# samuel-vitorino/lm.rs

Hardware: AMD Instinct MI355X
Metric: decode tok/s + %HBM-roofline, Llama-3.2-1B Q8_0 @1/2/4/8 MI355X vs CPU ref (higher is better)
Workload: dtype int8xint8->int32, f32 combine; 1 GPU; llama-3.2-1b Q8_0 (gs=128) greedy decode, 5-token synthetic prompt then 3164 tokens, batch 1; parallelism=single GPU, image_bytes=1274634496

## Files before the change

lm.rs_amd/csrc/lmrs_api.hip:

```cpp
#include <hip/hip_runtime.h>
#include <hip/hip_ext.h>
#include <rccl/rccl.h>
#include <math.h>
#include <stdio.h>
#include <stdlib.h>
#include <string.h>

#include <algorithm>
#include <chrono>
#include <string>
#include <vector>

#include "../../include/lmrs_hip.h"
#include "lmrs_device_math.h"
#include "lmrs_format.h"
#include "lmrs_kernels.h"
#include "lmrs_score.h"
#include "lmrs_switches.h"

using namespace lmrs;

static thread_local std::string g_err;
static int fail(const std::string& m) { g_err = m; return -1; }
#define HIP_OK(expr)                                                                                     \
// ... 3 lines not shown
    } while (0)

extern "C" const char* lmrs_last_error(void) { return g_err.c_str(); }
namespace lmrs { int text_fail(const char* msg) { return fail(msg); } }

namespace {

struct DevLayer {
    const void *wqkv, *wo, *w13, *w2;
    const float *sqkv, *so, *s13, *s2;
    const float *sqkvT = nullptr, *soT = nullptr, *s13T = nullptr, *s2T = nullptr;
    const float *rms_att, *rms_post_att, *rms_pre_ffn, *rms_post_ffn;
};

}
static int prefill_alloc(lmrs_ctx* c);

struct lmrs_ctx {
    lmrs_args args{};
    Layout lay;
    int device = 0;
    hipStream_t stream = nullptr;
    char* arena = nullptr; size_t arena_bytes = 0, arena_used = 0;
    std::vector<DevLayer> layers;
    const void *emb_q = nullptr, *cls_q = nullptr; const float *emb_s = nullptr, *cls_s = nullptr, *rms_final = nullptr;
    float *x = nullptr, *q = nullptr, *k_raw = nullptr, *att_out = nullptr, *h = nullptr, *logits = nullptr, *tmp = nullptr;
    float *part_val = nullptr; int* part_idx = nullptr;
    float *k_cache = nullptr, *v_cache = nullptr, *rope = nullptr;
    float* stage = nullptr; size_t stage_floats = 0;
    uint32_t* tokens = nullptr; DevState* st = nullptr;
    unsigned long long* dbg = nullptr; int dbg_node = 0;
    unsigned long long* samp_keys = nullptr; float* samp_pairs = nullptr; void* h_pairs = nullptr; int samp_cap = 0;
    float* h_logits = nullptr; uint32_t* h_tok = nullptr; DevState* h_st = nullptr; unsigned h_st_next = 0;
    hipGraphExec_t g_steps[7][2] = {}, g_layers = nullptr;
    float* att_S = nullptr; int att_split_pos = 0;
    float *pf_x = nullptr, *pf_q = nullptr, *pf_k = nullptr, *pf_ao = nullptr, *pf_h = nullptr, *pf_xs = nullptr, *pf_t = nullptr; int8_t* pf_xq = nullptr; float* pf_att = nullptr; size_t pf_att_cap = 0;
    bool pf_ready = false;
    char *pfx_att = nullptr, *pfx_h = nullptr, *pfx_x = nullptr; size_t pfb_att = 0, pfb_h = 0, pfb_x = 0; bool pfx_owned = false;
    bool tp_prefill = false;
    float* x2 = nullptr; bool gemma_fused = false;
    hipEvent_t ev0 = nullptr, ev1 = nullptr;
    Switches sw;
    std::vector<float*> scales_t;
    int att_dim = 0, kv_dim = 0, cls_grid = 0;
    int part_stride = 0;
    bool q4 = false, f32 = false;
    int rank = 0, world = 1;
    int att_full = 0;
    int dim_l = 0, hid_l = 0, voc_l = 0;
    int d0 = 0, h0 = 0, v0 = 0, a0 = 0;
    bool rep_out = true;
    bool cls_only = false;
    ncclComm_t comm = nullptr;
    bool eager = false;
    float* part = nullptr;
    bool qpay = false; char *gq_att = nullptr, *gq_h = nullptr; size_t blk_att = 0, blk_h = 0;
    bool p2p = false, p2p_ready = false; char* xarena = nullptr; size_t xarena_bytes = 0; char* peer_base[kMaxWorld] = {};
    unsigned *xflags = nullptr, *xseq = nullptr; int* xerr = nullptr; int ex_slot = 0; bool xarena_is_ipc[kMaxWorld] = {};
    double last_fill_ms = -1.0;
    bool err_queued = false;
    int* err = nullptr; int* h_err = nullptr;
    bool qkv_att = false; unsigned long long* gran = nullptr; unsigned* seq = nullptr; int qa_max_T = 0, qa_wave_T = 0;
    int multi_k = 1;
    bool cls_tail = false; unsigned long long* part_pk = nullptr; unsigned* cls_seq = nullptr;
    int inj_fail_connect = 0, inj_stall_seg = -1; long long inj_stall_ticks = 0;
    float* sc_logits = nullptr; int sc_rows = 0; ScorePart* sc_part = nullptr; double* sc_lp = nullptr; uint32_t* sc_idx = nullptr; char* h_sc = nullptr;
    unsigned long long* tk_cand = nullptr; uint32_t* tk_cnt = nullptr; uint32_t* tk_idx = nullptr; float* tk_val = nullptr; uint32_t* tk_rank = nullptr;
    char* h_tk = nullptr; int tk_rows = 0, tk_k = 0;

    template <class T> T* alloc(size_t count) {
        size_t bytes = (count * sizeof(T) + 255) & ~(size_t)255;
        if (arena_used + bytes > arena_bytes) return nullptr;
        T* p = reinterpret_cast<T*>(arena + arena_used); arena_used += bytes; return p;
    }
};

namespace {

__global__ void advance_pos_kernel(DevState* st, unsigned* seq) { st->pos += 1; st->step_count += 1; *seq += 1u; }
__global__ void stall_kernel(long long ticks) { const long long t0 = wall_clock64(); while (wall_clock64() - t0 < ticks) __builtin_amdgcn_s_sleep(32); }

size_t pad256(size_t b) { return (b + 255) & ~(size_t)255; }

constexpr int kPrefillTokens = 512;
bool prefill_tp_shapes_ok(const lmrs_ctx* c) {
    const lmrs_args& a = c->args;
    if (c->world < 1 || c->cls_only || c->f32 || c->sw.no_batched_prefill) return false;
    if (!c->rep_out && c->dim_l % 16) return false;
    if (a.q_type != LMRS_Q8_0 && a.q_type != LMRS_Q4_0) return false;
    if (c->att_dim % 128 || c->hid_l % 128) return false;
    if (!rows_prologue_supported((int)a.dim)) return false;
    if (a.model_type == LMRS_GEMMA) { if (a.head_size != 256 || a.dim != 2304) return false; }
    else if (a.head_size != 64 && a.head_size != 96 && a.head_size != 128) return false;
    return (c->att_dim + 2 * c->kv_dim) % 16 == 0 && c->kv_dim % 4 == 0 && a.dim % 16 == 0 && c->att_full % 128 == 0 && a.hidden_dim % 128 == 0;
}
size_t prefill_tp_block(size_t n_l) { return pad256((size_t)kPrefillTokens * n_l + (size_t)kPrefillTokens * (n_l / 128) * 4); }

struct StepForm { int qa_mode = 0, split_chunks = 0; };
struct PassForm { bool skinny = false; const RowTable* rows = nullptr; int max_T = 0; float *k_cache = nullptr, *v_cache = nullptr; RowView runs{}; float* qkv = nullptr; };
StepForm step_form_for(const lmrs_ctx* c, uint32_t pos, bool merged = true) {
    StepForm f;
    if (c->att_split_pos > 0 && (int)pos >= c->att_split_pos) {
        int b = 0;
        while (b < 3 && pos >= (1024u << b)) ++b;
        f.split_chunks = 4 << b;
    } else if (merged && c->qkv_att) f.qa_mode = (int)pos < c->qa_wave_T ? 2 : ((int)pos < c->qa_max_T ? 1 : 0);
    return f;
}
int split_scratch(lmrs_ctx* c, StepForm f) {
    if (!f.split_chunks || c->att_S) return 0;
    HIP_OK(hipMalloc(reinterpret_cast<void**>(&c->att_S), attention_split_scratch_floats(c->att_dim / (int)c->args.head_size, (int)c->args.seq_len) * 4));
    return 0;
}

void rope_terms(const lmrs_args& a, uint32_t p, uint32_t j, float* fcr, float* fci) {
    static const double short_factor[48] = {
        1.08, 1.1, 1.1300000000000001, 1.2800000000000002, 1.3100000000000003, 1.4500000000000004, 1.4500000000000004,
        1.9500000000000008, 2.030000000000001, 2.4299999999999926, 2.5699999999999896, 2.9499999999999815, 3.729999999999965,
        3.869999999999962, 4.189999999999955, 4.43999999999995, 4.6399999999999455, 4.979999999999938, 5.159999999999934,
        5.279999999999932, 5.759999999999922, 5.889999999999919, 5.889999999999919, 5.969999999999917, 6.089999999999915,
        6.2799999999999105, 6.7699999999999, 6.8899999999998975, 7.109999999999893, 7.129999999999892, 7.179999999999891,
        7.289999999999889, 7.339999999999888, 7.559999999999883, 7.619999999999882, 7.69999999999988, 7.879999999999876,
        7.879999999999876, 7.879999999999876, 7.939999999999875, 7.949999999999875, 7.979999999999874, 8.19999999999987,
        8.439999999999864, 8.469999999999864, 8.589999999999861, 8.809999999999857, 8.999999999999853};
    const uint32_t head_dim = j * 2;
    float freq = 1.0f / powf(a.rope_theta, (float)head_dim / (float)a.head_size);
    float scaling_factor = 1.0f;
    if (a.model_type == LMRS_LLAMA) {
        const float wavelen = (2.0f * 3.14159265358979323846f) / freq;
        const float factor = 32.0f, low_freq_factor = 1.0f, high_freq_factor = 4.0f, old_context_len = 8192.0f;
        const float low_freq_wavelen = old_context_len / low_freq_factor;
        const float high_freq_wavelen = old_context_len / high_freq_factor;
        if (wavelen > low_freq_wavelen) freq = freq / factor;
        else if (wavelen <= low_freq_wavelen && wavelen >= high_freq_wavelen) {
            const float smooth_factor = (old_context_len / wavelen - low_freq_factor) / (high_freq_factor - low_freq_factor);
            freq = (1.0f - smooth_factor) * freq / factor + smooth_factor * freq;
        }
    }
// ... 36 lines not shown
    HIP_OK(launch_gemv_f32(g, PRO_QUANT, gemma ? EPI_STORE : EPI_RESID, c->stream));
    set_launch_tag(7);
    if (gemma) HIP_OK(launch_addnorm(c->x, c->tmp, L.rms_post_att, a.dim, a.rms_norm_eps, c->stream));
    set_launch_tag(3);
    g.wq = L.w13; g.n = a.dim; g.o = 2 * a.hidden_dim; g.xin = c->x; g.rms_w = gemma ? L.rms_pre_ffn : L.rms_post_att; g.out = c->h;
    HIP_OK(launch_gemv_f32(g, PRO_RMS_QUANT, gemma ? EPI_GELU : EPI_SWIGLU, c->stream));
    set_launch_tag(4);
    g.wq = L.w2; g.n = a.hidden_dim; g.o = a.dim; g.xin = c->h; g.out = gemma ? c->tmp : c->x;
    HIP_OK(launch_gemv_f32(g, PRO_QUANT, gemma ? EPI_STORE : EPI_RESID, c->stream));
    set_launch_tag(7);
    if (gemma) HIP_OK(launch_addnorm(c->x, c->tmp, L.rms_post_ffn, a.dim, a.rms_norm_eps, c->stream));
    return 0;
}

int enqueue_layer(lmrs_ctx* c, StepForm f, int l) {
    if (c->f32) return enqueue_layer_f32(c, f, l);
    const lmrs_args& a = c->args;
    const DevLayer& L = c->layers[l];
    const bool gemma = a.model_type == LMRS_GEMMA;
    GemvArgs g{};
    g.q4 = c->q4; g.eps = a.rms_norm_eps; g.add_unit = gemma; g.st = c->st;
    g.att_dim = c->att_dim; g.kv_dim = c->kv_dim; g.seq_len = a.seq_len; g.layer = l;
    g.wq = L.wqkv; g.ws = L.sqkv; g.n = a.dim; g.o = c->att_dim + 2 * c->kv_dim;
    g.xin = c->x; g.rms_w = L.rms_att; g.out = c->q; g.k_raw = c->k_raw; g.v_cache = c->v_cache;
    g.att_dim = c->att_dim; g.kv_dim = c->kv_dim; g.seq_len = a.seq_len; g.layer = l;
    g.dbg = c->dbg ? c->dbg + 8 * (c->dbg_node++) : nullptr;
    set_launch_tag(0);
    const bool pending = c->gemma_fused && l > 0;
    if (pending) { g.xin = c->x2; g.delta = c->tmp; g.add_w = c->layers[l - 1].rms_post_ffn; g.xout = c->x; }
    AttnArgs t{};
    t.q = c->q; t.k_raw = c->k_raw; t.k_cache = c->k_cache; t.v_cache = c->v_cache; t.rope = c->rope; t.out = c->att_out;
    t.n_heads = a.n_heads; t.n_kv_heads = a.n_kv_heads; t.head_size = a.head_size; t.seq_len = a.seq_len; t.layer = l;
    t.gemma = gemma; t.st = c->st;
    if (f.qa_mode && !f.split_chunks) {
        g.gran = c->gran + (size_t)l * (c->att_dim + 2 * c->kv_dim); g.seq = c->seq;
        t.dbg = c->dbg ? c->dbg + 8 * (c->dbg_node++) : nullptr;
        HIP_OK(launch_qkv_attn(g, pending ? PRO_ADD_RMS_QUANT : PRO_RMS_QUANT, t, c->err, c->qa_max_T, f.qa_mode == 2, c->stream));
        g.gran = nullptr; g.seq = nullptr;
    } else {
    HIP_OK(launch_gemv(g, pending ? PRO_ADD_RMS_QUANT : PRO_RMS_QUANT, EPI_QKV, c->stream));
    t.dbg = c->dbg ? c->dbg + 8 * (c->dbg_node++) : nullptr;
    set_launch_tag(1);
    if (f.split_chunks) HIP_OK(launch_attention_split(t, c->att_S, f.split_chunks, c->stream));
    else HIP_OK(launch_attention(t, c->stream));
    }
    g.delta = nullptr; g.add_w = nullptr; g.xout = nullptr;
    g.wq = L.wo; g.ws = L.so; g.n = c->att_dim; g.o = a.dim; g.xin = c->att_out; g.out = gemma ? c->tmp : c->x;
    g.dbg = c->dbg ? c->dbg + 8 * (c->dbg_node++) : nullptr;
    set_launch_tag(2);
    HIP_OK(launch_gemv(g, PRO_QUANT, gemma ? EPI_STORE : EPI_RESID, c->stream));
    set_launch_tag(7);
    if (gemma && !c->gemma_fused) HIP_OK(launch_addnorm(c->x, c->tmp, L.rms_post_att, a.dim, a.rms_norm_eps, c->stream));
    g.wq = L.w13; g.ws = L.s13; g.n = a.dim; g.o = 2 * a.hidden_dim; g.xin = c->x; g.rms_w = gemma ? L.rms_pre_ffn : L.rms_post_att; g.out = c->h;
    g.dbg = c->dbg ? c->dbg + 8 * (c->dbg_node++) : nullptr;
    if (c->gemma_fused) { g.delta = c->tmp; g.add_w = L.rms_post_att; g.xout = c->x2; }
    set_launch_tag(3);
    HIP_OK(launch_gemv(g, c->gemma_fused ? PRO_ADD_RMS_QUANT : PRO_RMS_QUANT, gemma ? EPI_GELU : EPI_SWIGLU, c->stream));
    g.delta = nullptr; g.add_w = nullptr; g.xout = nullptr;
    g.wq = L.w2; g.ws = L.s2; g.n = a.hidden_dim; g.o = a.dim; g.xin = c->h; g.out = gemma ? c->tmp : c->x;
    g.dbg = c->dbg ? c->dbg + 8 * (c->dbg_node++) : nullptr;
    set_launch_tag(4);
    HIP_OK(launch_gemv(g, PRO_QUANT, gemma ? EPI_STORE : EPI_RESID, c->stream));
    set_launch_tag(7);
    if (gemma && !c->gemma_fused) HIP_OK(launch_addnorm(c->x, c->tmp, L.rms_post_ffn, a.dim, a.rms_norm_eps, c->stream));
    return 0;
}

// ... 223 lines not shown
        ++c->ex_slot;
        x.par_bytes = (int)e.par;
        if (e.qsrc) { x.qsrc = e.qsrc; x.qn = (int)e.qn; }
        set_launch_tag(8);
        HIP_OK(e.wide ? launch_exchange_copy_push(x, c->stream) : launch_exchange_push(x, c->stream));
        return 0;
    }
    if (!c->comm) return fail("this context is a member of a lock-step shard group: drive it with lmrs_group_forward");
    NCCL_OK(ncclAllGather(e.buf + (size_t)c->rank * e.stride, e.buf, e.stride, ncclUint8, c->comm, c->stream));
    return 0;
}

int capture(lmrs_ctx* c, StepForm f, bool full, hipGraphExec_t* out, int n_steps = 1) {
    hipGraph_t graph = nullptr;
    c->dbg_node = 0;
    HIP_OK(hipStreamBeginCapture(c->stream, hipStreamCaptureModeThreadLocal));
    int rc = 0;
    if (full) { for (int k = 0; k < n_steps && !rc; ++k) rc = c->world > 1 || c->comm ? enqueue_step_sharded(c, f) : enqueue_step(c, f); }
    else {
        for (uint32_t l = 0; l < c->args.n_layers && !rc; ++l) rc = enqueue_layer(c, f, (int)l);
        if (!rc) rc = enqueue_finish_residual(c);
        if (!rc) hipLaunchKernelGGL(advance_pos_kernel, dim3(1), dim3(1), 0, c->stream, c->st, c->seq);
    }
    hipError_t e = hipStreamEndCapture(c->stream, &graph);
    if (rc) { if (graph) (void)hipGraphDestroy(graph); return -1; }
    if (e != hipSuccess) return fail(std::string("hipStreamEndCapture: ") + hipGetErrorString(e));
    e = hipGraphInstantiate(out, graph, nullptr, nullptr, 0);
    (void)hipGraphDestroy(graph);
    if (e != hipSuccess) return fail(std::string("hipGraphInstantiate: ") + hipGetErrorString(e));
    return 0;
}

hipGraphExec_t step_graph(lmrs_ctx* c, StepForm f, int k = 1) {
    hipGraphExec_t& g = c->g_steps[f.split_chunks ? __builtin_ctz(f.split_chunks) + 1 : f.qa_mode][k > 1];
    if (!g && capture(c, f, true, &g, k)) g = nullptr;
    return g;
}
int replay_steps(lmrs_ctx* c, StepForm f, int k = 1) {
    hipGraphExec_t g = step_graph(c, f, k);
    if (!g) return -1;
    HIP_OK(hipGraphLaunch(g, c->stream));
    return 0;
}
hipGraphExec_t primary_graph(const lmrs_ctx* c) { return c->g_steps[step_form_for(c, 0).qa_mode][0]; }
void capture_sharded_step(lmrs_ctx* c) {
    if (!step_graph(c, step_form_for(c, 0))) { c->eager = true; (void)hipGetLastError(); g_err.clear(); }
}
void destroy_step_graphs(lmrs_ctx* c) {
    for (auto& forms : c->g_steps) for (hipGraphExec_t& g : forms) if (g) { (void)hipGraphExecDestroy(g); g = nullptr; }
}

int upload(lmrs_ctx* c, void* dst, const uint8_t* src, size_t bytes) {
    HIP_OK(hipMemcpyAsync(dst, src, bytes, hipMemcpyHostToDevice, c->stream));
    return 0;
}
int upload_interleaved(lmrs_ctx* c, void* dst, const uint8_t* src, size_t row_bytes, size_t rows, int phase) {
    HIP_OK(hipMemcpy2DAsync(static_cast<char*>(dst) + phase * row_bytes, 2 * row_bytes, src, row_bytes, row_bytes, rows,
                            hipMemcpyHostToDevice, c->stream));
    return 0;
}

constexpr unsigned kStateSlots = 16;
int set_state(lmrs_ctx* c, uint32_t pos, uint32_t prompt_end, int win_base = -1) {
    DevState* hs = c->h_st + (c->h_st_next++ % kStateSlots);
    hs->pos = (int)pos; hs->prompt_end = (int)prompt_end; hs->step_count = 0; hs->win_base = win_base;
    HIP_OK(hipMemcpyAsync(c->st, hs, sizeof(DevState), hipMemcpyHostToDevice, c->stream));
    if (c->qkv_att || c->cls_tail) HIP_OK(hipMemsetAsync(c->err, 0, 4, c->stream));
// ... 369 lines not shown
        std::vector<float> tab((size_t)a.seq_len * a.head_size);
        for (uint32_t p = 0; p < a.seq_len; ++p)
            for (uint32_t j = 0; j < half; ++j) rope_terms(a, p, j, &tab[((size_t)p * half + j) * 2], &tab[((size_t)p * half + j) * 2 + 1]);
        HCK(hipMemcpyAsync(c->rope, tab.data(), tab.size() * 4, hipMemcpyHostToDevice, c->stream));
        HCK(hipStreamSynchronize(c->stream));
    }
    HCK(hipHostMalloc(reinterpret_cast<void**>(&c->h_logits), V * 4, hipHostMallocDefault));
    HCK(hipHostMalloc(reinterpret_cast<void**>(&c->h_tok), ((size_t)a.seq_len + 8) * 4, hipHostMallocDefault));
    HCK(hipHostMalloc(reinterpret_cast<void**>(&c->h_st), kStateSlots * sizeof(DevState), hipHostMallocDefault));
    HCK(hipHostMalloc(reinterpret_cast<void**>(&c->h_err), 4, hipHostMallocDefault));
    CK(set_state(c, 0, 0));
    HCK(hipStreamSynchronize(c->stream));
    if (a.model_type == LMRS_GEMMA && !sharded && !f32w) {
        GemvArgs q{}; q.q4 = c->q4; q.n = a.dim; q.o = c->att_dim + 2 * c->kv_dim;
        GemvArgs f = q; f.o = 2 * a.hidden_dim;
        GemvArgs k = q; k.o = cls_rows(c); k.softcap_rows = (int)a.dim;
        c->gemma_fused = gemv_is_static(q, PRO_ADD_RMS_QUANT, EPI_QKV) && gemv_is_static(f, PRO_ADD_RMS_QUANT, EPI_GELU) &&
                         gemv_is_static(k, PRO_ADD_RMS_QUANT, EPI_CLS);
    }
    {
        GemvArgs g = cls_args(c);
        c->cls_grid = f32w ? gemv_f32_grid(g, EPI_CLS) : gemv_grid(g, c->gemma_fused ? PRO_ADD_RMS_QUANT : PRO_RMS_QUANT, EPI_CLS);
        c->part_stride = (2 * c->cls_grid + 3) & ~3;
    }
    if ((!sharded || (cls_only && !group_mode)) && !f32w && sw.qkv_att != 0) {
        GemvArgs q{}; q.q4 = c->q4; q.n = a.dim; q.o = c->att_dim + 2 * c->kv_dim;
        AttnArgs t{}; t.n_heads = a.n_heads; t.n_kv_heads = a.n_kv_heads; t.head_size = a.head_size; t.gemma = a.model_type == LMRS_GEMMA;
        c->qkv_att = qkv_attn_supported(q, PRO_RMS_QUANT, t) && (!c->gemma_fused || qkv_attn_supported(q, PRO_ADD_RMS_QUANT, t)) &&
                     !(a.model_type == LMRS_GEMMA && !c->gemma_fused);
        c->qa_max_T = a.seq_len < 1024 ? (int)a.seq_len : 1024;
        if (c->qkv_att && sw.qkv_att != 1) c->qa_wave_T = qkv_attn_wave_T((int)a.head_size);
        if (c->qa_wave_T > (int)a.seq_len) c->qa_wave_T = a.head_size == 64 && a.seq_len >= 128 ? (int)a.seq_len : 0;
    }
    if (!sharded) c->multi_k = sw.steps_per_graph;
    c->cls_tail = !sharded && !f32w && V < (1u << 20) - 1 && sw.cls_tail;
    if (!sharded) {
        CK(!step_graph(c, step_form_for(c, 0)));
        CK(capture(c, StepForm{}, false, &c->g_layers));
        if (!c->dbg || sw.att_split_pos_set) c->att_split_pos = sw.att_split_pos;
        if (!c->dbg && c->qkv_att) {
            for (int mode = 1; mode <= 2; ++mode) {
                if (mode == 2 && c->qa_wave_T <= 0) continue;
                if (mode == 1 && c->qa_wave_T >= c->qa_max_T) continue;
                CK(!step_graph(c, StepForm{mode, 0}));
                if (c->multi_k > 1) CK(!step_graph(c, StepForm{mode, 0}, c->multi_k));
            }
        }
    } else if (c->comm) {
        capture_sharded_step(c);
    }
    if (sharded) c->att_split_pos = sw.att_split_pos;
    if (c->tp_prefill && c->comm && (c->world > 1 || c->comm) && !c->cls_only) CK(prefill_alloc(c));
#undef CK
#undef HCK
    *out = c;
    if (bytes_consumed) *bytes_consumed = lay.end;
    return 0;
}

static void topk_free(lmrs_ctx* c) {
    for (void** p : {(void**)&c->tk_cand, (void**)&c->tk_cnt, (void**)&c->tk_idx, (void**)&c->tk_val, (void**)&c->tk_rank}) if (*p) { (void)hipFree(*p); *p = nullptr; }
    if (c->h_tk) { (void)hipHostFree(c->h_tk); c->h_tk = nullptr; }
    c->tk_rows = c->tk_k = 0;
}

extern "C" void lmrs_destroy(lmrs_ctx* c) {
// ... 1527 lines not shown
    return 0;
}

extern "C" int lmrs_debug_inject(lmrs_ctx* c, int what, int a, int b) {
    if (!c) return fail("ctx is NULL");
    if (what == 0) { c->inj_fail_connect = 1; return 0; }
    if (what == 1) {
        if (!(c->comm || c->p2p)) return fail("not a row-sharded context");
        HIP_OK(hipSetDevice(c->device));
        HIP_OK(hipStreamSynchronize(c->stream));
        destroy_step_graphs(c);
        c->eager = true; c->inj_stall_seg = a; c->inj_stall_ticks = (long long)b * 100;
        return 0;
    }
    return fail("unknown injection");
}

extern "C" int lmrs_debug_gemm_tile(uint32_t n, uint32_t o, uint32_t n_tok, int q4, int* tile_rows, int* tile_tokens, int* waves) {
    if (!tile_rows || !tile_tokens || !waves) return fail("NULL argument");
    if (n == 0 || n % 256 || o == 0 || o % 16 || n_tok == 0) return fail("lmrs_debug_gemm_tile: n must be a positive multiple of 256, o of 16");
    *tile_rows = *tile_tokens = *waves = 0;
    if (n_tok >= 48) { const GemmTile t = gemm_q8_ring_tile((int)n, (int)o, (int)n_tok, q4 != 0); *tile_rows = t.tm; *tile_tokens = t.tn; *waves = t.waves; }
    return 0;
}

extern "C" int lmrs_step_info(const lmrs_ctx* c, uint32_t pos, int* n_launches, double* algo_bytes) {
    if (!c) return fail("ctx is NULL");
    const lmrs_args& a = c->args;
    const double bpe = c->f32 ? 4.0 - 4.0 / 128.0 : (c->q4 ? 0.5 : 1.0), dim = a.dim, att = c->att_dim, kv = c->kv_dim, hid = a.hidden_dim, V = a.vocab_size, L = a.n_layers;
    const double n_norm = a.model_type == LMRS_GEMMA ? 4 : 2;
    double b = L * ((dim * att + 2 * dim * kv + att * dim + 3 * dim * hid) * (bpe + 4.0 / 128.0) + n_norm * dim * 4) + V * dim * (bpe + 4.0 / 128.0) +
               dim * 4 + L * 2 * kv * 4 * ((double)pos + 2);
    if (algo_bytes) *algo_bytes = b;
    if (n_launches) *n_launches = (a.model_type == LMRS_GEMMA && !c->gemma_fused ? 7 : (step_form_for(c, pos).qa_mode ? 4 : 5)) * (int)a.n_layers + (c->cls_tail ? 1 : 2);
    return 0;
}

namespace {
struct Scratch {
    std::vector<void*> p;
    ~Scratch() { for (void* q : p) (void)hipFree(q); }
    void* get(size_t bytes) { void* q = nullptr; if (hipMalloc(&q, bytes ? bytes : 4) != hipSuccess) return nullptr; p.push_back(q); return q; }
};
int op_begin(int device) {
    int ndev = 0;
    if (hipGetDeviceCount(&ndev) != hipSuccess || ndev == 0) return fail("no HIP device available (this library has no CPU fallback)");
    if (device < 0 || device >= ndev) return fail("bad device index");
    HIP_OK(hipSetDevice(device));
    return 0;
}
}

extern "C" int lmrs_op_matmul_q8(int device, float* xout, const int8_t* xq, const float* xs, const int8_t* wq, const float* ws,
                                 size_t n, size_t o, size_t gs, size_t sl) {
    if (op_begin(device)) return -1;
    if (gs != 128 || n % 128) return fail("group size must be 128 and n a multiple of it");
    Scratch S; const size_t G = n / 128;
    void *dx = S.get(sl * n), *dxs = S.get(sl * G * 4), *dw = S.get(o * n), *dws = S.get(o * G * 4), *dout = S.get(sl * o * 4);
    if (!dout) return fail("hipMalloc failed");
    HIP_OK(hipMemcpy(dx, xq, sl * n, hipMemcpyHostToDevice)); HIP_OK(hipMemcpy(dxs, xs, sl * G * 4, hipMemcpyHostToDevice));
    HIP_OK(hipMemcpy(dw, wq, o * n, hipMemcpyHostToDevice)); HIP_OK(hipMemcpy(dws, ws, o * G * 4, hipMemcpyHostToDevice));
    HIP_OK(hipMemset(dout, 0, sl * o * 4));
    const size_t o4 = o / 4 * 4;
    if (sl > 1 && n % 256 == 0 && o % 16 == 0) {
        GemmArgs g{}; g.wq = dw; g.ws = static_cast<float*>(dws); g.xq = static_cast<const int8_t*>(dx); g.xs = static_cast<const float*>(dxs);
        g.n = (int)n; g.o = (int)o; g.n_tok = (int)sl; g.out = static_cast<float*>(dout);
        HIP_OK(launch_gemm_q8(g, EPI_STORE, nullptr));
// ... 620 lines not shown
```

lm.rs_amd/csrc/lmrs_kernels.h:

```cpp
#pragma once
#include <hip/hip_runtime.h>
#include <stdint.h>

namespace lmrs {

struct DevState {
    int pos;
    int prompt_end;
    int step_count;
    int win_base;
};
constexpr int kWinPerQuery = -2;

enum Prologue { PRO_PREQ = 0, PRO_QUANT = 1, PRO_RMS_QUANT = 2, PRO_ADD_RMS_QUANT = 3 };
enum Epilogue { EPI_STORE = 0, EPI_RESID = 1, EPI_QKV = 2, EPI_SWIGLU = 3, EPI_CLS = 4, EPI_GELU = 5,
                EPI_VQKV = 6, EPI_BIAS_RESID = 7, EPI_BIAS_QGELU = 8,
                EPI_BIAS_GELU = 9, EPI_BIAS = 10,
                EPI_QKV_TAG = 11,
                EPI_SWIGLU_Q = 12, EPI_GELU_Q = 13 };

struct EmbedArgs {
    const void* emb_q; const float* emb_s; int q4;
    const uint32_t* tokens;
    float* x; int dim; float scale; int do_scale;
// ... 41 lines not shown
    int chain_spread;
};

struct AttnArgs {
    const float* q;
    const float* k_raw;
    float* k_cache;
    const float* v_cache;
    int chunk;
    const float* rope;
    float* out;
    int n_heads, n_kv_heads, head_size, seq_len, layer, gemma;
    unsigned long long* dbg;
    const DevState* st;
};

hipError_t launch_gemv(const GemvArgs& a, int pro, int epi, hipStream_t s, int grid_hint = 0);
void set_gemv_launch_events(hipEvent_t start, hipEvent_t stop);
void set_launch_event_pool(hipEvent_t* pairs, int n_pairs, int* tags = nullptr);
void set_launch_tag(int tag);
int launch_event_pool_used();
bool next_launch_events(hipEvent_t* a, hipEvent_t* b);
int gemv_grid(const GemvArgs& a, int pro, int epi);
bool gemv_is_static(const GemvArgs& a, int pro, int epi);
hipError_t launch_gemv_f32(const GemvArgs& a, int pro, int epi, hipStream_t s);
int gemv_f32_grid(const GemvArgs& a, int epi);
hipError_t launch_attention(const AttnArgs& a, hipStream_t s);
struct QkvAttnArgs { GemvArgs g; AttnArgs t; int* err; };
bool qkv_attn_supported(const GemvArgs& g, int pro, const AttnArgs& t);
int qkv_attn_wave_T(int head_size);
hipError_t launch_qkv_attn(const GemvArgs& g, int pro, const AttnArgs& t, int* err, int max_T, bool wave, hipStream_t s);
size_t attention_split_scratch_floats(int n_heads, int seq_len);
hipError_t launch_attention_split(const AttnArgs& a, float* S, int n_key_chunks, hipStream_t s);
hipError_t launch_embed(const EmbedArgs& a, hipStream_t s);
hipError_t launch_addvec(float* x, const float* d, int n, hipStream_t st);
hipError_t launch_addnorm(float* x, const float* delta, const float* w, int n, float eps, hipStream_t st);
hipError_t launch_argmax_final(const ArgmaxArgs& a, hipStream_t s);
hipError_t launch_dequant_rows(const void* q, const float* s, int q4, const uint32_t* tokens, int n_tok, int dim, float* out, hipStream_t st, float scale = 0.0f);

struct SampleArgs { float* logits; int n; float temperature; float* part; };
constexpr int kSampleGrid = 256;
hipError_t launch_sample_exps(const SampleArgs& a, hipStream_t s);
hipError_t launch_sample_topp_sort(const float* exps, int n, float sum, float cutoff, int N, unsigned long long* keys, unsigned* count, float* pairs_out, hipStream_t s);
int sample_sort_min_n();

struct SampleRow { float temperature, top_p, rnd; };
constexpr int kSampleRowsGrid = 64;
constexpr int kSampleRowsMax = 16;
struct SampleRowsArgs {
    float* rows; int n_rows, ld, n;
    const SampleRow* tab; const uint32_t* argmax;
    float* part; float* sum; unsigned* cnt; unsigned long long* out;
};
hipError_t launch_sample_rows(const SampleRowsArgs& a, hipStream_t s, int max_rows = kSampleRowsMax);

constexpr int kCandSortRowsMax = 64;
struct CandSortRows { unsigned row[kCandSortRowsMax]; unsigned n0[kCandSortRowsMax]; };
struct CandSortArgs { const unsigned long long* src; size_t ld; unsigned long long* keys; int N, n_rows; CandSortRows t; };
hipError_t launch_cand_sort(const CandSortArgs& a, hipStream_t s);

hipError_t launch_quantize(const float* x, void* q, float* s, int n, int q4, hipStream_t st);
hipError_t launch_quantize_rows(const float* x, int n, int n_tok, int q4, int8_t* q, float* s, hipStream_t st);
hipError_t launch_gather_rows(const char* blocks, size_t blk_stride, size_t s_off, int world, int n_l, int n_tok, int8_t* xq, float* xs, hipStream_t st, int xs_ld = 0);
hipError_t launch_scatter_rows(const char* blocks, size_t blk_stride, int world, int n_l, int n_tok, float* dst, int add, hipStream_t st);
hipError_t launch_rmsnorm(const float* x, const float* w, float* o, int n, float eps, int add_unit, hipStream_t st);
hipError_t launch_softmax(float* x, int n, hipStream_t st);
// ... 72 lines not shown
```

lm.rs_amd/csrc/lmrs_kernels.hip:

```cpp
#include <hip/hip_ext.h>
#include <mutex>
#include <map>
#include <set>
#include <tuple>
#include <utility>

#include "lmrs_device_math.h"
#include "lmrs_kernels.h"
#include "lmrs_stage.h"

namespace lmrs {

constexpr int kBlock = 256;


constexpr int kMaxP = 16;

template <int NP>
__device__ __forceinline__ void rmsnorm_inplace(float4 (&v)[NP], const float4 (&wv)[NP], int n, float eps,
                                                int add_unit, float* scratch) {
    const int t = threadIdx.x;
    const int P = (n + 1023) >> 10;
    const int JP = (n >> 3) + 4;
#pragma unroll
// ... 2054 lines not shown
            constexpr size_t wsm = HS == 64 ? (kMultiSmem > kPairSmem ? kMultiSmem : kPairSmem) : (QuadGeom<HS>::SMEM > WaveGeom<HS>::SMEM ? QuadGeom<HS>::SMEM : WaveGeom<HS>::SMEM);
            size_t smem = wsm > gsmem ? wsm : gsmem;
            if (smem > 64 * 1024) allow_big_lds(reinterpret_cast<const void*>(qkv_attn_kernel<N, L, PRO, Q4, HS, GEMMA, true>));
            grid = qkv_attn_grid(reinterpret_cast<const void*>(qkv_attn_kernel<N, L, PRO, Q4, HS, GEMMA, true>), smem, grid, a.t.n_heads);
            LMRS_LAUNCH_GRID((qkv_attn_kernel<N, L, PRO, Q4, HS, GEMMA, true>), dim3(grid), kBlock, smem, s, LMRS_HOT_OF(a.g), a);
            return hipGetLastError();
        }
    }
    if (wave) return hipErrorNotSupported;
    size_t smem = attention_smem(HS, qa_chunk(HS), max_T);
    if (gsmem > smem) smem = gsmem;
    if (smem > 64 * 1024) allow_big_lds(reinterpret_cast<const void*>(qkv_attn_kernel<N, L, PRO, Q4, HS, GEMMA, false>));
    grid = qkv_attn_grid(reinterpret_cast<const void*>(qkv_attn_kernel<N, L, PRO, Q4, HS, GEMMA, false>), smem, grid, a.t.n_heads);
    LMRS_LAUNCH_GRID((qkv_attn_kernel<N, L, PRO, Q4, HS, GEMMA, false>), dim3(grid), kBlock, smem, s, LMRS_HOT_OF(a.g), a);
    return hipGetLastError();
}

hipError_t launch_qkv_attn(const GemvArgs& g0, int pro, const AttnArgs& t0, int* err, int max_T, bool wave, hipStream_t s) {
    if (!qkv_attn_supported(g0, pro, t0) || !g0.gran || !g0.seq || !err) return hipErrorNotSupported;
    QkvAttnArgs a{g0, t0, err};
    a.g.order_barrier = a.g.chain_spread = 1;
    a.t.chunk = qa_chunk(t0.head_size);
    const StaticClass sc = static_class(a.g, pro, EPI_QKV);
    const int grid = t0.n_heads + gemv_grid(a.g, pro, EPI_QKV);
    const size_t gsmem = gemv_smem(a.g, pro);
#define X(n_, l_, p_, q_, hs_, gm_)                                                                                      \
    if (a.g.n == n_ && sc.L == l_ && pro == p_ && (a.g.q4 != 0) == q_ && t0.head_size == hs_ && (t0.gemma != 0) == gm_)  \
        return launch_qkv_attn_class<n_, l_, p_, q_, hs_, gm_>(a, grid, gsmem, max_T, wave, s);
    LMRS_QA_TABLE(X)
#undef X
    return hipErrorNotSupported;
}

template <int HS, bool GEMMA>
__global__ __launch_bounds__(kBlock) void attention_split_scores_kernel(const AttnArgs a, float* S) {
    __shared__ __attribute__((aligned(16))) float q[HS];
    __shared__ __attribute__((aligned(16))) float kn[HS];
    constexpr int half = HS / 2;
    const int h = blockIdx.x, tid = threadIdx.x;
    const int kv_mul = a.n_heads / a.n_kv_heads, kvh = h / kv_mul;
    const int pos = a.st->pos, T = pos + 1;
    const int t0 = blockIdx.y * kBlock;
    if (t0 >= T) return;
    const int SQ = a.seq_len;
    float* kT = att_k_head(a, kvh, HS);
    const __amdgpu_buffer_rsrc_t krs = __builtin_amdgcn_make_buffer_rsrc(kT, 0, HS * SQ * 4, 0x00020000);
    constexpr int KG = HS / 4 <= 32 ? HS / 4 : 16;
    const int t = t0 + tid, tc = t < T ? t : T - 1;
    f32x4v kk[KG];
    att_kload<KG>(kk, krs, tc * 16, 0, SQ);
    const bool mine = pos >= t0 && pos < t0 + kBlock;
    for (int j = tid; j < half; j += kBlock) {
        const float2 cs = *reinterpret_cast<const float2*>(a.rope + ((size_t)pos * half + j) * 2);
        const float2 rq = rope_rotate(a.q[h * HS + j], a.q[h * HS + j + half], cs.x, cs.y);
        q[j] = rq.x; q[j + half] = rq.y;
        if (mine) {
            const float2 rk = rope_rotate(a.k_raw[kvh * HS + j], a.k_raw[kvh * HS + j + half], cs.x, cs.y);
            kn[j] = rk.x; kn[j + half] = rk.y;
            k_store_pair(kT, SQ, pos, j, half, rk.x, rk.y);
        }
    }
    asm volatile("s_waitcnt vmcnt(0)" ::: "memory");
    lds_barrier();
    if (tc == pos) {
#pragma unroll
        for (int u = 0; u < KG; ++u) { const float4 t4 = reinterpret_cast<const float4*>(kn)[u]; kk[u] = f32x4v{t4.x, t4.y, t4.z, t4.w}; }
    }
    int wpos = pos;
    if constexpr (GEMMA) { const int wb = a.st->win_base; wpos = wb >= 0 ? wb : pos; }
    const float sqrt_hs = sqrtf((float)HS);
    float score = att_score_chain<HS, KG>(kk, krs, tc * 16, q, SQ);
    score = score / sqrt_hs;
    if constexpr (GEMMA) score = gemma_cap_window(score, wpos, t);
    if (t < T) S[(size_t)h * SQ + t] = score;
}

__device__ __forceinline__ float chain_rows16(float o, const float4* row, int nb) {
    float4 R[4][4];
#pragma unroll
    for (int k = 0; k < 3; ++k)
#pragma unroll
        for (int u = 0; u < 4; ++u) R[k][u] = row[k * 4 + u];
    for (int b = 0; b < nb; b += 4) {
#pragma unroll
        for (int k = 0; k < 4; ++k) {
            if (b + k >= nb) break;
#pragma unroll
            for (int u = 0; u < 4; ++u) R[(k + 3) & 3][u] = row[(b + k + 3) * 4 + u];
            asm volatile("" : "+v"(o) : : "memory");
#pragma unroll
            for (int u = 0; u < 4; ++u) { o = o + R[k][u].x; o = o + R[k][u].y; o = o + R[k][u].z; o = o + R[k][u].w; }
        }
    }
    return o;
}
template <int HS> struct SplitGeom {
    static constexpr int NSL = 4, HP = HS / NSL, HP4 = HP / 4, CHK = HS <= 128 ? 256 : 128, PITCH = CHK + 4;
    static constexpr int NLD = 3 * 64, NSLOT = (CHK * HP4 + NLD - 1) / NLD;
    static_assert(HP % 4 == 0 && HP <= 64, "dim slice");
};
template <int HS, bool GEMMA>
__global__ __launch_bounds__(kBlock) void attention_split_values_kernel(const AttnArgs a, const float* S) {
    using G = SplitGeom<HS>;
    constexpr int HP = G::HP, HP4 = G::HP4, CHK = G::CHK, PITCH = G::PITCH, NLD = G::NLD, NSLOT = G::NSLOT;
    extern __shared__ __attribute__((aligned(16))) char smem[];
    const int h = blockIdx.x, sl = blockIdx.y, tid = threadIdx.x, lane = tid & 63, wave = __builtin_amdgcn_readfirstlane(tid >> 6);
    const int kv_mul = a.n_heads / a.n_kv_heads, kvh = h / kv_mul, kv_dim = a.n_kv_heads * HS;
// ... 60 lines not shown
        }
        if (lane == 0) red[4] = sum;
    }
    lds_barrier();
    const float sum = red[4];
    if (stamp) a.dbg[4] = wall_clock64();
    for (int t = tid; t < T; t += kBlock) att[t] = att[t] / sum;
    lds_barrier();
    if (stamp) a.dbg[5] = wall_clock64();
    if (wave > 0) { vstore(0); if (nchunks > 1) vload(1); }
    lds_barrier();
    if (stamp) a.dbg[6] = wall_clock64();
    float o = 0.0f;
    for (int c = 0; c < nchunks; ++c) {
        if (wave == 0) {
          {
            const int t0 = c * CHK, ct = (T - t0) < CHK ? (T - t0) : CHK, nb = (ct + 15) >> 4;
            const float4* row = reinterpret_cast<const float4*>(tile + (c & 1) * HP * PITCH + (lane < HP ? lane : 0) * PITCH);
            o = chain_rows16(o, row, nb);
          }
        } else if (c + 1 < nchunks) {
            vstore(c + 1);
            if (c + 2 < nchunks) vload(c + 2);
        }
        lds_barrier();
    }
    if (wave == 0 && lane < HP) a.out[h * HS + sl * HP + lane] = o;
    if (stamp) a.dbg[7] = wall_clock64();
}

size_t attention_split_scratch_floats(int n_heads, int seq_len) { return (size_t)n_heads * seq_len; }

template <int HS, bool GEMMA>
static hipError_t launch_attention_split_hsg(const AttnArgs& a0, float* S, int n_key_chunks, hipStream_t s) {
    AttnArgs a = a0;
    using G = SplitGeom<HS>;
    a.chunk = G::CHK;
    const size_t smem = (size_t)(16 + 2 * G::HP * G::PITCH + ((a.seq_len + 3) & ~3) + 128) * 4;
    allow_big_lds(reinterpret_cast<const void*>(attention_split_values_kernel<HS, GEMMA>));
    LMRS_LAUNCH_GRID((attention_split_scores_kernel<HS, GEMMA>), dim3(a.n_heads, n_key_chunks), kBlock, 0, s, a, S);
    LMRS_LAUNCH_GRID((attention_split_values_kernel<HS, GEMMA>), dim3(a.n_heads, G::NSL), kBlock, smem, s, a, (const float*)S);
    return hipGetLastError();
}
hipError_t launch_attention_split(const AttnArgs& a, float* S, int n_key_chunks, hipStream_t s) {
#define AS(HS_) return a.gemma ? launch_attention_split_hsg<HS_, true>(a, S, n_key_chunks, s) : launch_attention_split_hsg<HS_, false>(a, S, n_key_chunks, s);
    switch (a.head_size) { case 64: AS(64) case 96: AS(96) case 128: AS(128) case 256: AS(256) default: return hipErrorInvalidValue; }
#undef AS
}

__global__ void embed_kernel(const EmbedArgs a) {
    const int pos = a.st->pos;
    const uint32_t token = a.tokens[pos];
    for (int i = blockIdx.x * blockDim.x + threadIdx.x; i < a.dim; i += gridDim.x * blockDim.x) {
        float v = dequant_elem(a.emb_q, a.emb_s, a.q4, (size_t)token * a.dim + i);
        if (a.do_scale) v = v * a.scale;
        a.x[i] = v;
    }
}

hipError_t launch_embed(const EmbedArgs& a, hipStream_t s) {
    hipLaunchKernelGGL(embed_kernel, dim3((a.dim + 255) / 256), dim3(256), 0, s, a);
    return hipGetLastError();
}

__global__ void dequant_rows_kernel(const void* q, const float* s, int q4, const uint32_t* tokens, int dim, float* out, float scale, int do_scale) {
    const uint32_t token = tokens[blockIdx.x];
    for (int i = threadIdx.x; i < dim; i += blockDim.x) {
        float v = dequant_elem(q, s, q4, (size_t)token * dim + i);
        if (do_scale) v = v * scale;
        out[(size_t)blockIdx.x * dim + i] = v;
    }
}

hipError_t launch_dequant_rows(const void* q, const float* s, int q4, const uint32_t* tokens, int n_tok, int dim, float* out, hipStream_t st, float scale) {
    hipLaunchKernelGGL(dequant_rows_kernel, dim3(n_tok), dim3(256), 0, st, q, s, q4, tokens, dim, out, scale, scale != 0.0f ? 1 : 0);
    return hipGetLastError();
}

// ... 643 lines not shown
```

lm.rs_amd/csrc/lmrs_switches.h:

```cpp
#pragma once
#include <stdlib.h>
#include <string.h>

namespace lmrs {

constexpr int kAttLdsKeys = 2048;

struct Switches {
    bool no_batched_prefill = false;
    int tokens_batch_min = 0;
    bool no_graph = false;
    bool debug_timeline = false;
    bool shard_f32_payload = false;
    bool group_p2p = false;
    bool att_long_batch_forms = false;
    bool vis_no_stray = false;
    int shard_plan = 0;
    bool shard_split_out = false;
    int qkv_att = -1;
    bool cls_tail = true;
    int att_split_pos = 384; bool att_split_pos_set = false;
    int att_lds_keys = kAttLdsKeys;
    int steps_per_graph = 4;
    size_t topp_sort_min = 4096;
    long long p2p_timeout_ms = 3000;
    int bsearch_flavour = 0;
};

inline Switches read_switches() {
    Switches s;
    const char* e;
    s.no_batched_prefill = getenv("LMRS_NO_BATCHED_PREFILL") != nullptr;
    if ((e = getenv("LMRS_TOKENS_BATCH_MIN"))) { const int k = atoi(e); s.tokens_batch_min = k < 2 ? 2 : k; }
    s.no_graph = getenv("LMRS_NO_GRAPH") != nullptr;
    s.debug_timeline = getenv("LMRS_DEBUG_TIMELINE") != nullptr;
    s.shard_f32_payload = getenv("LMRS_SHARD_F32_PAYLOAD") != nullptr;
    s.group_p2p = getenv("LMRS_GROUP_P2P") != nullptr;
    s.att_long_batch_forms = getenv("LMRS_ATT_LONG_BATCH_FORMS") != nullptr;
    s.vis_no_stray = getenv("LMRS_VIS_NO_STRAY") != nullptr;
    if ((e = getenv("LMRS_SHARD_PLAN"))) s.shard_plan = strcmp(e, "cls") ? 2 : 1;
    if ((e = getenv("LMRS_SHARD_SPLIT_OUT"))) s.shard_split_out = atoi(e) != 0;
    if ((e = getenv("LMRS_QKV_ATT"))) s.qkv_att = atoi(e);
    if ((e = getenv("LMRS_CLS_TAIL"))) s.cls_tail = atoi(e) != 0;
    if ((e = getenv("LMRS_ATT_SPLIT_POS"))) { s.att_split_pos = atoi(e); s.att_split_pos_set = true; }
    if ((e = getenv("LMRS_ATT_LDS_KEYS"))) s.att_lds_keys = atoi(e);
    if ((e = getenv("LMRS_STEPS_PER_GRAPH"))) { const int k = atoi(e); s.steps_per_graph = k < 1 ? 1 : (k > 64 ? 64 : k); }
    if ((e = getenv("LMRS_TOPP_DEVICE_SORT_MIN"))) s.topp_sort_min = (size_t)atol(e);
    if ((e = getenv("LMRS_P2P_TIMEOUT_MS"))) s.p2p_timeout_ms = atoll(e);
    if ((e = getenv("LMRS_BSEARCH_FLAVOUR"))) s.bsearch_flavour = atoi(e);
    return s;
}

}
```

Before: 1322 tok/s.

## Fuse QKV GEMV with split-attention score pass via granule polling

For long positions that use split attention, the QKV projection GEMV and the attention score kernel now run as a single launch. Score workgroups poll per-granule readiness tags written by the GEMV workgroups, so scoring can start as soon as q/k values are produced instead of waiting for a kernel boundary. The values pass stays a separate launch, which cuts one launch per layer. The cost is more complex in-kernel synchronisation, a risk of spinning or deadlock if the combined grid exceeds the resident capacity, and new graph slots for the merged forms.

```diff
diff --git a/lm.rs_amd/csrc/lmrs_api.hip b/lm.rs_amd/csrc/lmrs_api.hip
--- a/lm.rs_amd/csrc/lmrs_api.hip
+++ b/lm.rs_amd/csrc/lmrs_api.hip
@@ -59,8 +59,9 @@
     unsigned long long* dbg = nullptr; int dbg_node = 0;
     unsigned long long* samp_keys = nullptr; float* samp_pairs = nullptr; void* h_pairs = nullptr; int samp_cap = 0;
     float* h_logits = nullptr; uint32_t* h_tok = nullptr; DevState* h_st = nullptr; unsigned h_st_next = 0;
-    hipGraphExec_t g_steps[7][2] = {}, g_layers = nullptr;
+    hipGraphExec_t g_steps[11][2] = {}, g_layers = nullptr;
     float* att_S = nullptr; int att_split_pos = 0;
+    bool split_merged = false;
     float *pf_x = nullptr, *pf_q = nullptr, *pf_k = nullptr, *pf_ao = nullptr, *pf_h = nullptr, *pf_xs = nullptr, *pf_t = nullptr; int8_t* pf_xq = nullptr; float* pf_att = nullptr; size_t pf_att_cap = 0;
     bool pf_ready = false;
     char *pfx_att = nullptr, *pfx_h = nullptr, *pfx_x = nullptr; size_t pfb_att = 0, pfb_h = 0, pfb_x = 0; bool pfx_owned = false;
@@ -123,7 +124,7 @@
 }
 size_t prefill_tp_block(size_t n_l) { return pad256((size_t)kPrefillTokens * n_l + (size_t)kPrefillTokens * (n_l / 128) * 4); }
 
-struct StepForm { int qa_mode = 0, split_chunks = 0; };
+struct StepForm { int qa_mode = 0, split_chunks = 0; bool split_merged = false; };
 struct PassForm { bool skinny = false; const RowTable* rows = nullptr; int max_T = 0; float *k_cache = nullptr, *v_cache = nullptr; RowView runs{}; float* qkv = nullptr; };
 StepForm step_form_for(const lmrs_ctx* c, uint32_t pos, bool merged = true) {
     StepForm f;
@@ -131,6 +132,7 @@
         int b = 0;
         while (b < 3 && pos >= (1024u << b)) ++b;
         f.split_chunks = 4 << b;
+        f.split_merged = merged && c->split_merged;
     } else if (merged && c->qkv_att) f.qa_mode = (int)pos < c->qa_wave_T ? 2 : ((int)pos < c->qa_max_T ? 1 : 0);
     return f;
 }
@@ -233,7 +235,14 @@
     t.q = c->q; t.k_raw = c->k_raw; t.k_cache = c->k_cache; t.v_cache = c->v_cache; t.rope = c->rope; t.out = c->att_out;
     t.n_heads = a.n_heads; t.n_kv_heads = a.n_kv_heads; t.head_size = a.head_size; t.seq_len = a.seq_len; t.layer = l;
     t.gemma = gemma; t.st = c->st;
-    if (f.qa_mode && !f.split_chunks) {
+    if (f.split_chunks && f.split_merged) {
+        g.gran = c->gran + (size_t)l * (c->att_dim + 2 * c->kv_dim); g.seq = c->seq;
+        HIP_OK(launch_qkv_scores(g, pending ? PRO_ADD_RMS_QUANT : PRO_RMS_QUANT, t, c->att_S, c->err, f.split_chunks, c->sw.att_split_score_wgs, c->stream));
+        g.gran = nullptr; g.seq = nullptr;
+        t.dbg = c->dbg ? c->dbg + 8 * (c->dbg_node++) : nullptr;
+        set_launch_tag(1);
+        HIP_OK(launch_attention_split_values(t, c->att_S, c->stream));
+    } else if (f.qa_mode && !f.split_chunks) {
         g.gran = c->gran + (size_t)l * (c->att_dim + 2 * c->kv_dim); g.seq = c->seq;
         t.dbg = c->dbg ? c->dbg + 8 * (c->dbg_node++) : nullptr;
         HIP_OK(launch_qkv_attn(g, pending ? PRO_ADD_RMS_QUANT : PRO_RMS_QUANT, t, c->err, c->qa_max_T, f.qa_mode == 2, c->stream));
@@ -523,7 +532,7 @@
 }
 
 hipGraphExec_t step_graph(lmrs_ctx* c, StepForm f, int k = 1) {
-    hipGraphExec_t& g = c->g_steps[f.split_chunks ? __builtin_ctz(f.split_chunks) + 1 : f.qa_mode][k > 1];
+    hipGraphExec_t& g = c->g_steps[f.split_chunks ? __builtin_ctz(f.split_chunks) + (f.split_merged ? 5 : 1) : f.qa_mode][k > 1];
     if (!g && capture(c, f, true, &g, k)) g = nullptr;
     return g;
 }
@@ -959,6 +968,7 @@
         if (c->qkv_att && sw.qkv_att != 1) c->qa_wave_T = qkv_attn_wave_T((int)a.head_size);
         if (c->qa_wave_T > (int)a.seq_len) c->qa_wave_T = a.head_size == 64 && a.seq_len >= 128 ? (int)a.seq_len : 0;
     }
+    c->split_merged = c->qkv_att && !sharded && sw.att_split_merged;
     if (!sharded) c->multi_k = sw.steps_per_graph;
     c->cls_tail = !sharded && !f32w && V < (1u << 20) - 1 && sw.cls_tail;
     if (!sharded) {
@@ -2552,7 +2562,9 @@
     double b = L * ((dim * att + 2 * dim * kv + att * dim + 3 * dim * hid) * (bpe + 4.0 / 128.0) + n_norm * dim * 4) + V * dim * (bpe + 4.0 / 128.0) +
                dim * 4 + L * 2 * kv * 4 * ((double)pos + 2);
     if (algo_bytes) *algo_bytes = b;
-    if (n_launches) *n_launches = (a.model_type == LMRS_GEMMA && !c->gemma_fused ? 7 : (step_form_for(c, pos).qa_mode ? 4 : 5)) * (int)a.n_layers + (c->cls_tail ? 1 : 2);
+    const StepForm f = step_form_for(c, pos);
+    const int att_launches = f.split_chunks ? (f.split_merged ? 2 : 3) : (f.qa_mode ? 1 : 2);
+    if (n_launches) *n_launches = ((a.model_type == LMRS_GEMMA && !c->gemma_fused ? 5 : 3) + att_launches) * (int)a.n_layers + (c->cls_tail ? 1 : 2);
     return 0;
 }
 
diff --git a/lm.rs_amd/csrc/lmrs_kernels.h b/lm.rs_amd/csrc/lmrs_kernels.h
--- a/lm.rs_amd/csrc/lmrs_kernels.h
+++ b/lm.rs_amd/csrc/lmrs_kernels.h
@@ -97,6 +97,8 @@
 hipError_t launch_qkv_attn(const GemvArgs& g, int pro, const AttnArgs& t, int* err, int max_T, bool wave, hipStream_t s);
 size_t attention_split_scratch_floats(int n_heads, int seq_len);
 hipError_t launch_attention_split(const AttnArgs& a, float* S, int n_key_chunks, hipStream_t s);
+hipError_t launch_qkv_scores(const GemvArgs& g, int pro, const AttnArgs& t, float* S, int* err, int n_key_chunks, int max_score_wgs, hipStream_t s);
+hipError_t launch_attention_split_values(const AttnArgs& a, const float* S, hipStream_t s);
 hipError_t launch_embed(const EmbedArgs& a, hipStream_t s);
 hipError_t launch_addvec(float* x, const float* d, int n, hipStream_t st);
 hipError_t launch_addnorm(float* x, const float* delta, const float* w, int n, float eps, hipStream_t st);
diff --git a/lm.rs_amd/csrc/lmrs_kernels.hip b/lm.rs_amd/csrc/lmrs_kernels.hip
--- a/lm.rs_amd/csrc/lmrs_kernels.hip
+++ b/lm.rs_amd/csrc/lmrs_kernels.hip
@@ -2110,16 +2110,13 @@
     return hipErrorNotSupported;
 }
 
-template <int HS, bool GEMMA>
-__global__ __launch_bounds__(kBlock) void attention_split_scores_kernel(const AttnArgs a, float* S) {
-    __shared__ __attribute__((aligned(16))) float q[HS];
-    __shared__ __attribute__((aligned(16))) float kn[HS];
+template <int HS, bool GEMMA, bool TAG>
+__device__ __forceinline__ void split_scores_item(const AttnArgs& a, float* S, int h, int t0, int pos, float* q, float* kn, const AttTag& tg = AttTag()) {
+    static_assert(!TAG || HS <= kBlock, "granule polling: one value of each vector per lane");
     constexpr int half = HS / 2;
-    const int h = blockIdx.x, tid = threadIdx.x;
+    const int tid = threadIdx.x;
     const int kv_mul = a.n_heads / a.n_kv_heads, kvh = h / kv_mul;
-    const int pos = a.st->pos, T = pos + 1;
-    const int t0 = blockIdx.y * kBlock;
-    if (t0 >= T) return;
+    const int T = pos + 1;
     const int SQ = a.seq_len;
     float* kT = att_k_head(a, kvh, HS);
     const __amdgpu_buffer_rsrc_t krs = __builtin_amdgcn_make_buffer_rsrc(kT, 0, HS * SQ * 4, 0x00020000);
@@ -2128,17 +2125,40 @@
     f32x4v kk[KG];
     att_kload<KG>(kk, krs, tc * 16, 0, SQ);
     const bool mine = pos >= t0 && pos < t0 + kBlock;
+    float2 cs_tag = make_float2(0.f, 0.f);
+    if constexpr (TAG) {
+        cs_tag = *reinterpret_cast<const float2*>(a.rope + ((size_t)pos * half + (tid < half ? tid : 0)) * 2);
+        if (tid < HS) {
+            const unsigned long long* gp3[3];
+            granules_of(tg, h, kvh, HS, tid, gp3);
+            if (mine) {
+                const unsigned long long* gp[2] = {gp3[0], gp3[1]};
+                unsigned long long xg[2];
+                poll_granules<2>(gp, tg, a.layer, xg);
+                q[tid] = __uint_as_float((unsigned)xg[0]); kn[tid] = __uint_as_float((unsigned)xg[1]);
+            } else {
+                const unsigned long long* gp[1] = {gp3[0]};
+                unsigned long long xg[1];
+                poll_granules<1>(gp, tg, a.layer, xg);
+                q[tid] = __uint_as_float((unsigned)xg[0]);
+            }
+        }
+        lds_barrier();
+    }
     for (int j = tid; j < half; j += kBlock) {
-        const float2 cs = *reinterpret_cast<const float2*>(a.rope + ((size_t)pos * half + j) * 2);
-        const float2 rq = rope_rotate(a.q[h * HS + j], a.q[h * HS + j + half], cs.x, cs.y);
+        float2 cs;
+        if constexpr (TAG) cs = cs_tag; else cs = *reinterpret_cast<const float2*>(a.rope + ((size_t)pos * half + j) * 2);
+        const float q0 = TAG ? q[j] : a.q[h * HS + j], q1 = TAG ? q[j + half] : a.q[h * HS + j + half];
+        const float2 rq = rope_rotate(q0, q1, cs.x, cs.y);
         q[j] = rq.x; q[j + half] = rq.y;
         if (mine) {
-            const float2 rk = rope_rotate(a.k_raw[kvh * HS + j], a.k_raw[kvh * HS + j + half], cs.x, cs.y);
+            const float k0 = TAG ? kn[j] : a.k_raw[kvh * HS + j], k1 = TAG ? kn[j + half] : a.k_raw[kvh * HS + j + half];
+            const float2 rk = rope_rotate(k0, k1, cs.x, cs.y);
             kn[j] = rk.x; kn[j + half] = rk.y;
             k_store_pair(kT, SQ, pos, j, half, rk.x, rk.y);
         }
     }
-    asm volatile("s_waitcnt vmcnt(0)" ::: "memory");
+    if (!TAG || (mine && HS / 4 > KG)) asm volatile("s_waitcnt vmcnt(0)" ::: "memory");
     lds_barrier();
     if (tc == pos) {
 #pragma unroll
@@ -2151,6 +2171,70 @@
     score = score / sqrt_hs;
     if constexpr (GEMMA) score = gemma_cap_window(score, wpos, t);
     if (t < T) S[(size_t)h * SQ + t] = score;
+}
+
+template <int HS, bool GEMMA>
+__global__ __launch_bounds__(kBlock) void attention_split_scores_kernel(const AttnArgs a, float* S) {
+    __shared__ __attribute__((aligned(16))) float q[HS];
+    __shared__ __attribute__((aligned(16))) float kn[HS];
+    const int pos = a.st->pos;
+    const int t0 = blockIdx.y * kBlock;
+    if (t0 > pos) return;
+    split_scores_item<HS, GEMMA, false>(a, S, blockIdx.x, t0, pos, q, kn);
+}
+
+template <int N, int L, int PRO, bool Q4, int HS, bool GEMMA>
+__global__ __launch_bounds__(kBlock) void qkv_scores_kernel(LMRS_HOT_PARAMS, const QkvAttnArgs a0, float* S, const int n_gemv) {
+    extern __shared__ __attribute__((aligned(16))) char smem[];
+    QkvAttnArgs a = a0;
+    a.g = with_hot(a0.g, h_xin, h_wq, h_ws, h_rms_w, h_st, h_seq, h_out); a.t.st = h_st;
+    if ((int)blockIdx.x < n_gemv) {
+        gemv_static_body<N, L, PRO, EPI_QKV_TAG, kBlock, Q4>(a.g, smem, (int)blockIdx.x, n_gemv);
+        return;
+    }
+    const int pos = a.t.st->pos;
+    const AttTag tg{a.g.gran, *a.g.seq + 1u, a.g.att_dim, a.g.kv_dim, a.err};
+    float* q = reinterpret_cast<float*>(smem);
+    float* kn = q + HS;
+    const int nh = a.t.n_heads, nkv = a.t.n_kv_heads;
+    const int n_items = nh * (pos / kBlock + 1), n_score = (int)gridDim.x - n_gemv;
+    bool further = false;
+    for (int it = (int)blockIdx.x - n_gemv; it < n_items; it += n_score, further = true) {
+        const int chunk = it / nh, hq = it - chunk * nh, bq = hq / nkv, br = hq - bq * nkv;
+        if (further) lds_barrier();
+        split_scores_item<HS, GEMMA, true>(a.t, S, br * (nh / nkv) + bq, chunk * kBlock, pos, q, kn, tg);
+    }
+}
+
+template <int N, int L, int PRO, bool Q4, int HS, bool GEMMA>
+static hipError_t launch_qkv_scores_class(const QkvAttnArgs& a, float* S, int n_gemv, int n_score, size_t smem, int max_score_wgs, hipStream_t s) {
+    const void* fn = reinterpret_cast<const void*>(qkv_scores_kernel<N, L, PRO, Q4, HS, GEMMA>);
+    if (smem > 64 * 1024) allow_big_lds(fn);
+    const int cap = resident_grid_cap(fn, smem);
+    if (cap > a.t.n_heads + 64 && n_gemv + n_score > cap) {
+        const int floor_wgs = a.t.n_heads > cap / 4 ? a.t.n_heads : cap / 4;
+        if (n_score > floor_wgs) n_score = cap - n_gemv > floor_wgs ? cap - n_gemv : floor_wgs;
+        if (n_gemv + n_score > cap) n_gemv = cap - n_score;
+    }
+    if (max_score_wgs > 0 && n_score > max_score_wgs) n_score = max_score_wgs;
+    LMRS_LAUNCH_GRID((qkv_scores_kernel<N, L, PRO, Q4, HS, GEMMA>), dim3(n_gemv + n_score), kBlock, smem, s, LMRS_HOT_OF(a.g), a, S, n_gemv);
+    return hipGetLastError();
+}
+
+hipError_t launch_qkv_scores(const GemvArgs& g0, int pro, const AttnArgs& t0, float* S, int* err, int n_key_chunks, int max_score_wgs, hipStream_t s) {
+    if (!qkv_attn_supported(g0, pro, t0) || !g0.gran || !g0.seq || !err || !S || n_key_chunks <= 0) return hipErrorNotSupported;
+    QkvAttnArgs a{g0, t0, err};
+    a.g.order_barrier = a.g.chain_spread = 1;
+    const StaticClass sc = static_class(a.g, pro, EPI_QKV);
+    const int n_gemv = gemv_grid(a.g, pro, EPI_QKV);
+    size_t smem = gemv_smem(a.g, pro);
+    if (smem < (size_t)2 * t0.head_size * 4) smem = (size_t)2 * t0.head_size * 4;
+#define X(n_, l_, p_, q_, hs_, gm_)                                                                                      \
+    if (a.g.n == n_ && sc.L == l_ && pro == p_ && (a.g.q4 != 0) == q_ && t0.head_size == hs_ && (t0.gemma != 0) == gm_)  \
+        return launch_qkv_scores_class<n_, l_, p_, q_, hs_, gm_>(a, S, n_gemv, t0.n_heads * n_key_chunks, smem, max_score_wgs, s);
+    LMRS_QA_TABLE(X)
+#undef X
+    return hipErrorNotSupported;
 }
 
 __device__ __forceinline__ float chain_rows16(float o, const float4* row, int nb) {
@@ -2277,18 +2361,29 @@
 size_t attention_split_scratch_floats(int n_heads, int seq_len) { return (size_t)n_heads * seq_len; }
 
 template <int HS, bool GEMMA>
-static hipError_t launch_attention_split_hsg(const AttnArgs& a0, float* S, int n_key_chunks, hipStream_t s) {
+static hipError_t launch_split_values_hsg(const AttnArgs& a0, const float* S, hipStream_t s) {
     AttnArgs a = a0;
     using G = SplitGeom<HS>;
     a.chunk = G::CHK;
     const size_t smem = (size_t)(16 + 2 * G::HP * G::PITCH + ((a.seq_len + 3) & ~3) + 128) * 4;
     allow_big_lds(reinterpret_cast<const void*>(attention_split_values_kernel<HS, GEMMA>));
+    LMRS_LAUNCH_GRID((attention_split_values_kernel<HS, GEMMA>), dim3(a.n_heads, G::NSL), kBlock, smem, s, a, S);
+    return hipGetLastError();
+}
+template <int HS, bool GEMMA>
+static hipError_t launch_attention_split_hsg(const AttnArgs& a0, float* S, int n_key_chunks, hipStream_t s) {
+    AttnArgs a = a0;
+    a.chunk = SplitGeom<HS>::CHK;
     LMRS_LAUNCH_GRID((attention_split_scores_kernel<HS, GEMMA>), dim3(a.n_heads, n_key_chunks), kBlock, 0, s, a, S);
-    LMRS_LAUNCH_GRID((attention_split_values_kernel<HS, GEMMA>), dim3(a.n_heads, G::NSL), kBlock, smem, s, a, (const float*)S);
-    return hipGetLastError();
+    return launch_split_values_hsg<HS, GEMMA>(a0, S, s);
 }
 hipError_t launch_attention_split(const AttnArgs& a, float* S, int n_key_chunks, hipStream_t s) {
 #define AS(HS_) return a.gemma ? launch_attention_split_hsg<HS_, true>(a, S, n_key_chunks, s) : launch_attention_split_hsg<HS_, false>(a, S, n_key_chunks, s);
+    switch (a.head_size) { case 64: AS(64) case 96: AS(96) case 128: AS(128) case 256: AS(256) default: return hipErrorInvalidValue; }
+#undef AS
+}
+hipError_t launch_attention_split_values(const AttnArgs& a, const float* S, hipStream_t s) {
+#define AS(HS_) return a.gemma ? launch_split_values_hsg<HS_, true>(a, S, s) : launch_split_values_hsg<HS_, false>(a, S, s);
     switch (a.head_size) { case 64: AS(64) case 96: AS(96) case 128: AS(128) case 256: AS(256) default: return hipErrorInvalidValue; }
 #undef AS
 }
diff --git a/lm.rs_amd/csrc/lmrs_switches.h b/lm.rs_amd/csrc/lmrs_switches.h
--- a/lm.rs_amd/csrc/lmrs_switches.h
+++ b/lm.rs_amd/csrc/lmrs_switches.h
@@ -20,6 +20,8 @@
     int qkv_att = -1;
     bool cls_tail = true;
     int att_split_pos = 384; bool att_split_pos_set = false;
+    bool att_split_merged = true;
+    int att_split_score_wgs = 0;
     int att_lds_keys = kAttLdsKeys;
     int steps_per_graph = 4;
     size_t topp_sort_min = 4096;
@@ -43,6 +45,8 @@
     if ((e = getenv("LMRS_QKV_ATT"))) s.qkv_att = atoi(e);
     if ((e = getenv("LMRS_CLS_TAIL"))) s.cls_tail = atoi(e) != 0;
     if ((e = getenv("LMRS_ATT_SPLIT_POS"))) { s.att_split_pos = atoi(e); s.att_split_pos_set = true; }
+    if ((e = getenv("LMRS_ATT_SPLIT_MERGED"))) s.att_split_merged = atoi(e) != 0;
+    if ((e = getenv("LMRS_ATT_SPLIT_SCORE_WGS"))) { const int k = atoi(e); s.att_split_score_wgs = k < 0 ? 0 : k; }
     if ((e = getenv("LMRS_ATT_LDS_KEYS"))) s.att_lds_keys = atoi(e);
     if ((e = getenv("LMRS_STEPS_PER_GRAPH"))) { const int k = atoi(e); s.steps_per_graph = k < 1 ? 1 : (k > 64 ? 64 : k); }
     if ((e = getenv("LMRS_TOPP_DEVICE_SORT_MIN"))) s.topp_sort_min = (size_t)atol(e);
```

Result: faster. 1388 tok/s (median of 6 runs) (+5.0%).
